# nkkrnkl/category-agnostic-pose-estimation

Hardware: AMD Instinct MI355X
Metric: episodes/sec (1-shot, 256x256, 17kpt) training step (higher is better)
Workload: dtype f32 storage/accumulate, GEMMs as bf16x3 split (3 bf16 MFMAs per product); 1 GPU; configs[1]: 1-shot training step (fwd+loss+bwd+clip+AdamW at learning rate 0, dropout on), 256x256, 17 kpt, ResNet-50 + deformable transformer, 16 episodes x 2 queries per GPU; episodes_per_gpu=16, queries_per_episode=2, image_size=256, global_batch_episodes=16, parallelism=dp1, weights=random init (no checkpoint offline)

## Files before the change

category-agnostic-pose-estimation_amd/hip/functional.py:

```python
import contextlib
import ctypes
import os

import torch

from . import lib, ops


class Runtime:
    rng = None
    direct_grad = False
    use_side_stream = os.environ.get("CAPE_SIDE_STREAM", "1") == "1"
    side = None
    on_param_grad = []
    capture_keep = None

    pending = []
    side_dirty = False

    defer_wgrad = os.environ.get("CAPE_DEFER_WGRAD", "1") == "1"
    wgrad_group = int(os.environ.get("CAPE_WGRAD_GROUP", "12"))
    wq = {}
    wq_total = 0
    wq_notify = []
# ... 1059 lines not shown
        ref = _c(ref)
        ctx.save_for_backward(ref)
        return ops.query_sine_fwd(ref).view(*ref.shape[:-1], 256)

    @staticmethod
    def backward(ctx, d_out):
        (ref,) = ctx.saved_tensors
        return ops.query_sine_bwd(_c(d_out).view(-1, 256), ref).view_as(ref)


def query_sine(ref):
    return QuerySineFn.apply(ref)


class RefineFn(torch.autograd.Function):
    @staticmethod
    def forward(ctx, delta, ref):
        delta, ref = _c(delta), _c(ref)
        out = ops.refine_fwd(delta, ref)
        ctx.save_for_backward(out, ref)
        return out

    @staticmethod
    def backward(ctx, d_new):
        out, ref = ctx.saved_tensors
        d_delta, d_ref = ops.refine_bwd(_c(d_new), out, ref)
        return d_delta, d_ref


def refine(delta, ref):
    return RefineFn.apply(delta, ref)


class SigmoidFn(torch.autograd.Function):
    @staticmethod
    def forward(ctx, x):
        y = ops.sigmoid_fwd(_c(x))
        ctx.save_for_backward(y)
        return y

    @staticmethod
    def backward(ctx, dy):
        (y,) = ctx.saved_tensors
        return ops.sigmoid_bwd(_c(dy), y)


def sigmoid(x):
    return SigmoidFn.apply(x)


class RefScaleFn(torch.autograd.Function):

    @staticmethod
    def forward(ctx, ref, valid_ratios):
        ref, vr = _c(ref), _c(valid_ratios)
        N, Lq, _ = ref.shape
        L = vr.shape[1]
        ctx.save_for_backward(vr)
        ctx.meta = (N, Lq, L)
        return ops.ref_scale_fwd(ref, vr, Lq, L).view(N, Lq, L, 2)

    @staticmethod
    def backward(ctx, d):
        (vr,) = ctx.saved_tensors
        N, Lq, L = ctx.meta
        return ops.ref_scale_bwd(_c(d), vr, Lq, L).view(N, Lq, 2), None
# ... 193 lines not shown
```

category-agnostic-pose-estimation_amd/hip/lib.py:

```python
import ctypes
import os

import torch

from ctypes import POINTER, c_char_p, c_float, c_int, c_int32, c_int64, c_longlong, c_size_t, c_uint32, c_uint64, c_uint8, c_void_p

_HERE = os.path.dirname(os.path.abspath(__file__))
LIB_PATH = os.environ.get("CAPE_HIP_LIB", os.path.join(_HERE, "..", "csrc", "libcape_hip.so"))
LIB_PATH = os.path.abspath(LIB_PATH)

if not os.path.exists(LIB_PATH):
    raise ImportError(
        f"libcape_hip.so not found at {LIB_PATH}; build it with `python -c 'import __graft_entry__ as g; g.build()'` "
        "(or `make -C category-agnostic-pose-estimation_amd/csrc`).  There is no CPU fallback.")
try:
    _lib = ctypes.CDLL(LIB_PATH)
except OSError as e:
    raise ImportError(f"cannot load {LIB_PATH}: {e}") from e

_lib.cape_last_error.restype = c_char_p
_lib.cape_abi_version.restype = c_int


class GemmDesc(ctypes.Structure):
# ... 100 lines not shown
    "cape_msda_bwd": [P, P, P, P, P, P, P, P, P, I, I, I, I, I, P],
    "cape_msda_bwd_ex": [P, P, P, P, P, P, P, P, P, I, I, I, I, I, I, P],
    "cape_msda_bwd_atomic": [P, P, P, P, P, P, P, P, P, I, I, I, I, I, P],
    "cape_attn_fwd": [P, P, P, P, P, LL, LL, LL, LL, LL, LL, LL, LL, I, I, I, I, F, I, I, P, F, P, U32, P],
    "cape_attn_bwd": [P, P, P, P, P, P, P, P, P, LL, LL, LL, LL, LL, LL, LL, LL, I, I, I, I, F, I, I, P, F, P, U32, P],
    "cape_flash_attn_fwd": [P, P, P, P, P, LL, LL, LL, LL, LL, LL, LL, LL, I, I, I, I, F, I, I, P, F, P, U32, P],
    "cape_flash_attn_bwd": [P, P, P, P, P, P, P, P, P, P, LL, LL, LL, LL, LL, LL, LL, LL, I, I, I, I, F, I, I, P, F, P, U32, P],
    "cape_attn_softmax_fwd": [P, P, P, I, I, I, I, F, I, I, P, F, P, U32, P],
    "cape_attn_softmax_bwd": [P, P, I, I, I, I, F, F, P, U32, P],
    "cape_add_f32": [P, P, P, LL, P],
    "cape_level_embed_add": [P, P, P, P, I, I, I, I, P],
    "cape_add_n_f32": [POINTER(c_void_p), I, P, LL, P],
    "cape_add_n_rows_f32": [POINTER(c_void_p), POINTER(c_longlong), I, P, LL, LL, I, P],
    "cape_augment_batch": [P, I, I, I, P, P, P],
    "cape_gelu_f32": [P, P, LL, P],
    "cape_support_masks": [P, P, P, I, I, I, P],
    "cape_interleave2x2_f32": [POINTER(c_void_p), P, P, I, I, I, I, P],
    "cape_gelu_bwd_f32": [P, P, P, LL, P],
    "cape_scale_residual_bwd_f32": [P, P, P, P, P, LL, I, P],
    "cape_scale_residual_f32": [P, P, P, P, LL, I, P],
    "cape_nchw_to_nhwc": [P, P, I, I, I, I, I, P],
    "cape_bn_fold": [P, P, P, P, F, P, P, I, P],
    "cape_maxpool3x3s2_nhwc": [P, P, I, I, I, I, P],
    "cape_bn_relu_bwd": [P, P, P, P, P, LL, I, I, P],
    "cape_affine_act_f32": [P, P, P, P, LL, I, I, P],
    "cape_relu_drop_bwd": [P, P, P, LL, F, P],
    "cape_pos_sine_level": [P, P, P, P, LL, I, I, I, I, P],
    "cape_token_embed_fwd": [P, P, P, P, P, P, P, P, P, P, LL, I, I, P],
    "cape_token_embed_bwd": [P, P, P, P, P, P, P, P, P, P, LL, I, I, I, P],
    "cape_query_sine_fwd": [P, P, P, LL, P],
    "cape_query_sine_bwd": [P, P, P, P, I, LL, P],
    "cape_refine_fwd": [P, P, P, LL, P],
    "cape_refine_bwd": [P, P, P, P, P, I, LL, P],
    "cape_sigmoid_fwd": [P, P, LL, P],
    "cape_sigmoid_bwd": [P, P, P, I, LL, P],
    "cape_ref_scale_fwd": [P, P, P, LL, I, I, P],
    "cape_ref_scale_bwd": [P, P, P, I, LL, I, I, P],
    "cape_support_embed_fwd": [P, P, P, P, P, P, P, I, I, I, P],
    "cape_support_embed_bwd": [P, P, P, P, P, I, I, I, P],
    "cape_adjacency": [P, P, P, P, I, I, P],
    "cape_gcn_aggregate_fwd": [P, P, P, I, I, I, P],
    "cape_gcn_aggregate_bwd": [P, P, P, P, I, I, I, P],
    "cape_zero_rows": [P, P, LL, I, P],
    "cape_legacy_coord_embed_fwd": [P, P, P, P, I, I, P],
    "cape_legacy_coord_embed_bwd": [P, P, P, P, P, P, P, I, I, P],
    "cape_support_edge_info_fwd": [P, P, P, P, LL, P, P, P, I, I, I, P],
    "cape_support_edge_info_bwd": [P, LL, P, P, P, I, I, P],
    "cape_pe_dropout_fwd": [P, P, P, I, I, I, F, P, U32, P],
    "cape_pe_dropout_bwd": [P, P, LL, F, P, U32, P],
    "cape_loss_fwd_bwd": [P, P, P, P, P, P, F, F, F, P, P, P, P, I, LL, P],
    "cape_sumsq": [P, LL, P, P],
    "cape_adamw_step": [P, P, P, P, LL, F, F, F, F, F, F, P, I, P, P, P],
    "cape_step_increment": [P, P],
    "cape_step_guard": [P, P, I, P, I, F, P, P, P, P, P, I, I, P],
    "cape_adamw_step_guarded": [P, P, P, P, LL, F, F, F, F, F, F, P, I, P, P, P, P],
    "cape_decode_next_tokens": [P, P, P, P, P, P, I, I, I, I, I, I, P],
    "cape_decode_advance": [P, LL, P, LL, P, P, P, I, I, I, I, I, I, I, P, I, I, P, P, P],
    "cape_decode_linear": [POINTER(DecodeLinearDesc), P],
    "cape_decode_tail": [POINTER(DecodeTailDesc), P],
    "cape_decode_step": [POINTER(DecodeStepDesc), P],
}
EXPORTS = ["cape_last_error", "cape_abi_version", "cape_groupnorm_workspace_bytes", "cape_packed_weight_bytes"] + list(_SIGS)
_lib.cape_packed_weight_bytes.argtypes = [I, I]
_lib.cape_packed_weight_bytes.restype = c_size_t
_lib.cape_groupnorm_workspace_bytes.argtypes = [I, I, I]
_lib.cape_groupnorm_workspace_bytes.restype = c_size_t
# ... 24 lines not shown
```

category-agnostic-pose-estimation_amd/hip/ops.py:

```python
import ctypes
import math
import os
import weakref

import torch

from . import lib

_F32 = torch.float32


_raw_stream = getattr(torch._C, "_cuda_getCurrentRawStream", None)
_raw_device = getattr(torch._C, "_cuda_getDevice", None)


_side = [None]


def raw_current_stream():
    if _raw_stream is not None and _raw_device is not None:
        return _raw_stream(_raw_device())
    return torch.cuda.current_stream().cuda_stream


# ... 552 lines not shown
         batch=(N * H, H, Q.stride(0), 32, K.stride(0), 32, H * Lq * Lk, Lq * Lk))
    P = torch.empty_like(S)
    Pd = torch.empty_like(S) if dropout_p > 0 else None
    lib.call("cape_attn_softmax_fwd", _p(S), _p(P), _p(Pd), N, H, Lq, Lk, float(scale), mask_mode, causal_offset, _p(kpm),
             float(dropout_p), _rng_ptr(rng, dropout_p), rng_stream, _stream())
    Pu = Pd if Pd is not None else P
    O = torch.empty(N, Lq, H * 32, dtype=_F32, device=dev)
    gemm(Pu, V, O, Lq, 32, Lk, a_mode=0, b_mode=1, lda=Lk, ldb=_ld(V), ldc=H * 32,
         batch=(N * H, H, H * Lq * Lk, Lq * Lk, V.stride(0), 32, Lq * H * 32, 32))
    return O, P, Pu


def attn_mm_bwd(dO, Q, K, V, P, Pu, dQ, dK, dV, N, H, Lq, Lk, scale, dropout_p=0.0, rng=None, rng_stream=0):
    blk, img = Lq * Lk, H * Lq * Lk
    gemm(Pu, dO, dV, Lk, 32, Lq, a_mode=1, b_mode=1, lda=Lk, ldb=H * 32, ldc=_ld(dV),
         batch=(N * H, H, img, blk, Lq * H * 32, 32, dV.stride(0), 32))
    dS = torch.empty(N, H, Lq, Lk, dtype=_F32, device=dO.device)
    gemm(dO, V, dS, Lq, Lk, 32, lda=H * 32, ldb=_ld(V), ldc=Lk,
         batch=(N * H, H, Lq * H * 32, 32, V.stride(0), 32, img, blk))
    lib.call("cape_attn_softmax_bwd", _p(P), _p(dS), N, H, Lq, Lk, float(scale), float(dropout_p),
             _rng_ptr(rng, dropout_p), rng_stream, _stream())
    gemm(dS, K, dQ, Lq, 32, Lk, a_mode=0, b_mode=1, lda=Lk, ldb=_ld(K), ldc=_ld(dQ),
         batch=(N * H, H, img, blk, K.stride(0), 32, dQ.stride(0), 32))
    gemm(dS, Q, dK, Lk, 32, Lq, a_mode=1, b_mode=1, lda=Lk, ldb=_ld(Q), ldc=_ld(dK),
         batch=(N * H, H, img, blk, Q.stride(0), 32, dK.stride(0), 32))


def attn_route(N, H, Lq, Lk, flash=False):
    if flash and flash_attn_ok(N, H, Lq, Lk):
        return "flash"
    return "mm" if attn_mm_ok(N, H, Lq, Lk) else "scalar"


_ATTN_LAUNCHERS = {"scalar": (attn_fwd, attn_bwd), "flash": (flash_attn_fwd, flash_attn_bwd)}


def attn_core_fwd(route, Q, K, V, N, H, Lq, Lk, scale, mask_mode=0, causal_offset=0, kpm=None, dropout_p=0.0, rng=None, rng_stream=0):
    if route == "mm":
        O, P, Pu = attn_mm_fwd(Q, K, V, N, H, Lq, Lk, scale, mask_mode, causal_offset, kpm, dropout_p, rng, rng_stream)
        return O, (P, Pu)
    O, lse = _ATTN_LAUNCHERS[route][0](Q, K, V, N, H, Lq, Lk, scale, mask_mode, causal_offset, kpm, dropout_p, rng, rng_stream)
    return O, (lse,)


def attn_core_bwd(route, saved, dO, Q, K, V, O, dQ, dK, dV, N, H, Lq, Lk, scale, mask_mode=0, causal_offset=0, kpm=None, dropout_p=0.0,
                  rng=None, rng_stream=0):
    if route == "mm":
        attn_mm_bwd(dO, Q, K, V, *saved, dQ, dK, dV, N, H, Lq, Lk, scale, dropout_p, rng, rng_stream)
    else:
        _ATTN_LAUNCHERS[route][1](dO, Q, K, V, O, *saved, dQ, dK, dV, N, H, Lq, Lk, scale, mask_mode, causal_offset, kpm, dropout_p,
                                  rng, rng_stream)


def add(a, b):
    _chk(a, "add.a"); _chk(b, "add.b")
    assert a.shape == b.shape
    out = torch.empty_like(a)
    lib.call("cape_add_f32", _p(a), _p(b), _p(out), a.numel(), _stream())
    return out


def add_n(tensors):
    k = len(tensors)
    assert 1 <= k <= 8
    for t in tensors:
        _chk(t, "add_n.src")
# ... 206 lines not shown
    R = seqs[0].numel()
    lib.call("cape_token_embed_bwd", _p(d_out), *[_p(s) for s in seqs], *[_p(d) for d in deltas], _p(d_table), R, C, V,
             int(pad_idx), _stream())


def query_sine_fwd(ref):
    _chk(ref, "qsine.ref")
    R = ref.numel() // 2
    out = torch.empty(R, 256, dtype=_F32, device=ref.device)
    lib.call("cape_query_sine_fwd", _p(ref), _p(dim_t(ref.device)), _p(out), R, _stream())
    return out


def query_sine_bwd(d_out, ref):
    _chk(d_out, "qsine_bwd.d_out")
    d_ref = torch.empty_like(ref)
    lib.call("cape_query_sine_bwd", _p(d_out), _p(ref), _p(dim_t(ref.device)), _p(d_ref), 0, ref.numel() // 2, _stream())
    return d_ref


def refine_fwd(delta, ref):
    _chk(delta, "refine.delta"); _chk(ref, "refine.ref")
    assert delta.shape == ref.shape
    out = torch.empty_like(ref)
    lib.call("cape_refine_fwd", _p(delta), _p(ref), _p(out), ref.numel(), _stream())
    return out


def refine_bwd(d_new, new_ref, ref):
    _chk(d_new, "refine_bwd.d_new")
    d_delta, d_ref = torch.empty_like(ref), torch.empty_like(ref)
    lib.call("cape_refine_bwd", _p(d_new), _p(new_ref), _p(ref), _p(d_delta), _p(d_ref), 0, ref.numel(), _stream())
    return d_delta, d_ref


def sigmoid_fwd(x):
    _chk(x, "sigmoid.x")
    y = torch.empty_like(x)
    lib.call("cape_sigmoid_fwd", _p(x), _p(y), x.numel(), _stream())
    return y


def sigmoid_bwd(dy, y):
    _chk(dy, "sigmoid_bwd.dy")
    dx = torch.empty_like(y)
    lib.call("cape_sigmoid_bwd", _p(dy), _p(y), _p(dx), 0, y.numel(), _stream())
    return dx


def ref_scale_fwd(ref, valid_ratios, rows_per_image, L):
    _chk(ref, "ref_scale.ref"); _chk(valid_ratios, "ref_scale.vr")
    R = ref.numel() // 2
    out = torch.empty(R, L, 2, dtype=_F32, device=ref.device)
    lib.call("cape_ref_scale_fwd", _p(ref), _p(valid_ratios), _p(out), R, rows_per_image, L, _stream())
    return out


def ref_scale_bwd(d_in, valid_ratios, rows_per_image, L):
    _chk(d_in, "ref_scale_bwd.d_in")
    R = d_in.numel() // (2 * L)
    d_ref = torch.empty(R, 2, dtype=_F32, device=d_in.device)
    lib.call("cape_ref_scale_bwd", _p(d_in), _p(valid_ratios), _p(d_ref), 0, R, rows_per_image, L, _stream())
    return d_ref


def support_embed_fwd(coords, W0, b0, pe1d, N, P, C=256):
# ... 368 lines not shown
```

category-agnostic-pose-estimation_amd/models/deformable_transformer_v2.py:

```python
import copy
import math
import os

import numpy as np
import torch
from torch import nn
from torch.nn.init import normal_

from ..hip import functional as HF
from ..hip import ops
from .deformable_transformer import (DeformableTransformerEncoder, DeformableTransformerEncoderLayer, MSDeformAttn)
from ..util.misc import cached_zero_mask
from .kv_cache import KVCache, VCache

_ONES_VR = {}
_FUSED_SELF_ATTN = os.environ.get("CAPE_DEC_SELF_ATTN_NODE", "1") == "1"


def Embedding(num_embeddings, embedding_dim, padding_idx=None, zero_init=False):
    m = nn.Embedding(num_embeddings, embedding_dim, padding_idx=padding_idx)
    nn.init.normal_(m.weight, mean=0, std=embedding_dim ** -0.5)
    if padding_idx is not None:
        nn.init.constant_(m.weight[padding_idx], 0)
    if zero_init:
# ... 149 lines not shown
        return HF.token_embed(self.token_embed.weight, self.pad_idx, seq11, seq21, seq12, seq22,
                              delta_x1, delta_x2, delta_y1, delta_y2)

    def _query_pos(self, reference_points):
        qs = HF.query_sine(reference_points)
        qp = HF.linear(qs, self.pos_trans.weight, self.pos_trans.bias)
        return HF.add_layernorm(qp, None, self.pos_trans_norm.weight, self.pos_trans_norm.bias)

    def _mlp(self, mlp, x):
        n = len(mlp.layers)
        for i, layer in enumerate(mlp.layers):
            x = HF.linear(x, layer.weight, layer.bias, relu=(i < n - 1))
        return x

    def forward(self, reference_points, src, geo, src_valid_ratios, padding_rows_u8=None, seq_kwargs=None,
                support_features=None, support_mask=None):
        if support_features is None:
            support_features = getattr(self, "support_features", None)
        if support_mask is None:
            support_mask = getattr(self, "support_mask", None)
        kpm = ops.as_u8(support_mask) if (support_features is not None and support_mask is not None) else None
        output = self._seq_embed(seq11=seq_kwargs["seq11"], seq12=seq_kwargs["seq12"], seq21=seq_kwargs["seq21"],
                                 seq22=seq_kwargs["seq22"], delta_x1=seq_kwargs["delta_x1"], delta_x2=seq_kwargs["delta_x2"],
                                 delta_y1=seq_kwargs["delta_y1"], delta_y2=seq_kwargs["delta_y2"])
        hs, refs, clss = [], [], []
        nl = len(self.layers)
        mems = HF.fanout(src, nl)
        sups = HF.fanout(support_features, nl) if support_features is not None else (None,) * nl
        for lid, layer in enumerate(self.layers):
            r_scale, r_sine, r_ref = HF.fanout(reference_points, 3)
            ref_in = HF.ref_scale(r_scale, src_valid_ratios)
            query_pos = self._query_pos(r_sine)
            output = layer(output, query_pos, ref_in, mems[lid], geo, padding_rows_u8, sups[lid], kpm)
            o_mlp, o_cls, o_hs, output = HF.fanout(output, 4)
            delta = self._mlp(self.coords_embed[lid], o_mlp)
            reference_points, r_keep = HF.fanout(HF.refine(delta, r_ref), 2)
            cls = HF.linear(o_cls, self.class_embed[lid].weight, self.class_embed[lid].bias)
            hs.append(o_hs); refs.append(r_keep); clss.append(cls)
        return hs, torch.stack(refs), torch.stack(clss)

    @torch.no_grad()
    def decode_step(self, tok, delta, ref_step, geo, valid_ratios, step, caches):
        N = tok.shape[1]
        output = ops.token_embed_fwd(self.token_embed.weight, [tok[0], tok[2], tok[1], tok[3]],
                                     [delta[0], delta[1], delta[2], delta[3]]).view(N, 1, -1)
        ref = ref_step
        for lid, layer in enumerate(self.layers):
            ref_in = ops.ref_scale_fwd(ref, valid_ratios, 1, geo.L).view(N, 1, geo.L, 2)
            qs = ops.query_sine_fwd(ref)
            qp = torch.empty(N, 256, dtype=torch.float32, device=ref.device)
            ops.gemm(qs, self.pos_trans.weight, qp, N, 256, 256, bias=self.pos_trans.bias)
            qp, _, _, _ = ops.add_layernorm_fwd(qp, None, self.pos_trans_norm.weight, self.pos_trans_norm.bias)
            output = layer.decode_step(output, qp.view(N, 1, 256), ref_in, geo, step, caches[lid])
            x = output.view(N, 256)
            mlp = self.coords_embed[lid].layers
            for i, l in enumerate(mlp):
                y = torch.empty(N, l.weight.shape[0], dtype=torch.float32, device=x.device)
                ops.gemm(x, l.weight, y, N, l.weight.shape[0], l.weight.shape[1], bias=l.bias, relu=(i < len(mlp) - 1))
                x = y
            ref = ops.refine_fwd(x.view(N, 1, 2), ref)
        ce = self.class_embed[-1]
        cls = torch.empty(N, ce.weight.shape[0], dtype=torch.float32, device=ref.device)
        ops.gemm(output.view(N, 256), ce.weight, cls, N, ce.weight.shape[0], 256, bias=ce.bias)
        return output, ref, cls


class DeformableTransformer(nn.Module):
    def __init__(self, d_model=256, nhead=8, num_encoder_layers=6, num_decoder_layers=6, dim_feedforward=1024, dropout=0.1,
                 activation="relu", poly_refine=True, return_intermediate_dec=False, aux_loss=False, num_feature_levels=4,
                 dec_n_points=4, enc_n_points=4, query_pos_type="none", vocab_size=None, seq_len=1024,
# ... 87 lines not shown
```

include/cape_hip.h:

```cpp
#ifndef CAPE_HIP_H
#define CAPE_HIP_H

#include <stddef.h>
#include <stdint.h>

#ifdef __cplusplus
extern "C" {
#endif

typedef void* cape_stream_t;

const char* cape_last_error(void);
int cape_abi_version(void);

int cape_rng_advance(uint64_t* rng_state, cape_stream_t stream);

int cape_stream_fork(cape_stream_t main_stream, cape_stream_t side_stream);
int cape_stream_join(cape_stream_t main_stream, cape_stream_t side_stream);

typedef struct {
  int M, N, K;
  int a_mode, b_mode;
  const float* A; long long lda;
  const float* B; long long ldb;
// ... 166 lines not shown
int cape_scale_residual_f32(const float* x, const float* y, const float* gamma, float* out, long long rows, int C,
                            cape_stream_t stream);
int cape_gelu_bwd_f32(const float* x, const float* g, float* dx, long long n, cape_stream_t stream);
int cape_scale_residual_bwd_f32(const float* g, const float* y, const float* gamma, float* dy, float* dgamma, long long rows, int C,
                                cape_stream_t stream);
int cape_nchw_to_nhwc(const float* x, float* out, int N, int C, int H, int W, int Cp, cape_stream_t stream);
int cape_bn_fold(const float* w, const float* b, const float* rm, const float* rv, float eps,
                 float* scale, float* shift, int C, cape_stream_t stream);
int cape_maxpool3x3s2_nhwc(const float* x, float* out, int N, int H, int W, int C, cape_stream_t stream);
int cape_bn_relu_bwd(const float* dy, const float* y, const float* scale, float* d_pre, float* d_res,
                     long long rows, int C, int relu, cape_stream_t stream);
int cape_affine_act_f32(float* x, const float* scale, const float* bias, const float* residual, long long rows, int C, int relu,
                        cape_stream_t stream);
int cape_relu_drop_bwd(const float* dh, const float* h, float* d_pre, long long n, float inv_keep,
                       cape_stream_t stream);
int cape_pos_sine_level(const uint8_t* mask, const float* level_embed_l, const float* dim_t, float* out,
                        long long out_image_stride, int N, int h, int w, int C, cape_stream_t stream);

int cape_token_embed_fwd(const float* table, const int64_t* s11, const int64_t* s21, const int64_t* s12,
                         const int64_t* s22, const float* dx1, const float* dx2, const float* dy1,
                         const float* dy2, float* out, long long R, int C, int vocab, cape_stream_t stream);
int cape_token_embed_bwd(const float* d_out, const int64_t* s11, const int64_t* s21, const int64_t* s12,
                         const int64_t* s22, const float* dx1, const float* dx2, const float* dy1,
                         const float* dy2, float* d_table, long long R, int C, int vocab, int pad_idx,
                         cape_stream_t stream);

int cape_query_sine_fwd(const float* ref, const float* dim_t, float* out, long long R, cape_stream_t stream);
int cape_query_sine_bwd(const float* d_out, const float* ref, const float* dim_t, float* d_ref, int accumulate, long long R,
                        cape_stream_t stream);

int cape_refine_fwd(const float* delta, const float* ref, float* new_ref, long long n, cape_stream_t stream);
int cape_refine_bwd(const float* d_new, const float* new_ref, const float* ref, float* d_delta,
                    float* d_ref, int accumulate_ref, long long n, cape_stream_t stream);
int cape_sigmoid_fwd(const float* x, float* y, long long n, cape_stream_t stream);
int cape_sigmoid_bwd(const float* dy, const float* y, float* dx, int accumulate, long long n,
                     cape_stream_t stream);
int cape_ref_scale_fwd(const float* ref, const float* valid_ratios, float* ref_in, long long R,
                       int rows_per_image, int L, cape_stream_t stream);
int cape_ref_scale_bwd(const float* d_ref_in, const float* valid_ratios, float* d_ref, int accumulate,
                       long long R, int rows_per_image, int L, cape_stream_t stream);

int cape_support_embed_fwd(const float* coords, const float* W0, const float* b0, const float* pe1d,
                           const float* dim_t, float* h, float* pe, int N, int P, int C, cape_stream_t stream);
int cape_support_embed_bwd(const float* d_h, const float* h, const float* coords, float* dW0, float* db0,
                           int N, int P, int C, cape_stream_t stream);
int cape_adjacency(const int* edges, const int* edge_start, const uint8_t* mask, float* adj, int N, int P,
                   cape_stream_t stream);
int cape_support_masks(const uint8_t* mask, uint8_t* kpm, uint8_t* zero, int N, int P, int pad_rows, cape_stream_t stream);
int cape_gcn_aggregate_fwd(const float* y, const float* adj, float* out, int N, int P, int C,
                           cape_stream_t stream);
int cape_gcn_aggregate_bwd(const float* d_out, const float* out, const float* adj, float* d_y, int N,
                           int P, int C, cape_stream_t stream);
int cape_zero_rows(float* x, const uint8_t* rowmask, long long rows, int C, cape_stream_t stream);

int cape_legacy_coord_embed_fwd(const float* coords, const float* W0, const float* b0, float* h, int R, int C, cape_stream_t stream);
int cape_legacy_coord_embed_bwd(const float* d_h, const float* h, const float* coords, const float* W0, float* dW0, float* db0,
                                float* d_coords, int R, int C, cape_stream_t stream);
int cape_support_edge_info_fwd(const int* edges, const int* edge_start, const float* E, float* out, long long ldo, float* scale,
                               uint8_t* has, float* deg, int N, int P, int C, cape_stream_t stream);
int cape_support_edge_info_bwd(const float* g, long long ldg, const float* scale, const uint8_t* has, float* dE, int R, int C,
                               cape_stream_t stream);
int cape_pe_dropout_fwd(const float* x, const float* pe, float* out, int R, int P, int C, float dropout_p, const uint64_t* rng_state,
                        uint32_t rng_stream, cape_stream_t stream);
int cape_pe_dropout_bwd(const float* g, float* dx, long long total, float dropout_p, const uint64_t* rng_state, uint32_t rng_stream,
                        cape_stream_t stream);

// ... 54 lines not shown
```

Measured before the change: 648.3 episodes/s.

## Fuse decoder coord MLP, refine and class heads into single kernels

Adds fused HIP forward and backward kernels that run the decoder's per-layer 3-layer coordinate MLP, the inverse-sigmoid refine, and the class linear head in one launch each. Activations stay in LDS as bf16 hi/lo planes between the MFMA stages instead of going through separate GEMM and elementwise launches. The goal is to cut per-layer launch count and intermediate global memory traffic. It adds routing logic and packed-weight lookup, and small-weight gradients are summed with atomics.

```diff
diff --git a/category-agnostic-pose-estimation_amd/csrc/dec_chain.hip b/category-agnostic-pose-estimation_amd/csrc/dec_chain.hip
--- /dev/null
+++ b/category-agnostic-pose-estimation_amd/csrc/dec_chain.hip
@@ -0,0 +1,407 @@
+#include "gemm_common.h"
+
+namespace {
+
+constexpr int DC_UNIT = 64;
+constexpr int DC_C = 256;
+constexpr int DC_KS = DC_C / 16;
+constexpr int DC_LD = DC_C + 8;
+constexpr int DC_PLANE = DC_UNIT * DC_LD;
+constexpr int DC_IMG = 2 * DC_PLANE;
+constexpr int DC_FLD = DC_C + 4;
+constexpr int DC_SMALL = DC_UNIT * 8 + 5 * DC_C;
+constexpr size_t DC_LDS_BYTES = (size_t)2 * DC_IMG * 2 + (size_t)DC_SMALL * 4;
+static_assert((size_t)DC_UNIT * DC_FLD * 4 <= (size_t)DC_IMG * 2, "an fp32 unit fits in one image");
+static_assert(DC_LDS_BYTES <= 160 * 1024, "LDS of one CU");
+
+#define DC_PIN() asm volatile("" ::: "memory")
+__device__ __forceinline__ unsigned dc_opaque_zero() {
+  unsigned z = 0;
+  asm volatile("" : "+s"(z));
+  return z;
+}
+
+__device__ __forceinline__ int roff16(int i) { return (i & 3) + 8 * (i >> 2); }
+
+__device__ __forceinline__ void load_frags(bf16x8 (&bhi)[DC_KS], bf16x8 (&blo)[DC_KS], const unsigned short* pack, int grp, int lane) {
+  const char* bp = reinterpret_cast<const char*>(pack) + ((size_t)grp * (DC_KS * 2 * 1024) + dc_opaque_zero());
+  const unsigned lo = 16u * (unsigned)lane;
+#pragma unroll
+  for (int s = 0; s < DC_KS; ++s) {
+    bhi[s] = __builtin_bit_cast(bf16x8, *reinterpret_cast<const uint4*>(bp + (2 * s + 0) * 1024 + lo));
+    blo[s] = __builtin_bit_cast(bf16x8, *reinterpret_cast<const uint4*>(bp + (2 * s + 1) * 1024 + lo));
+  }
+}
+
+__device__ __forceinline__ f32x16 stage_mma(const unsigned short* img, int half, int r, int h, const bf16x8 (&bhi)[DC_KS],
+                                            const bf16x8 (&blo)[DC_KS], int single) {
+  f32x16 acc;
+#pragma unroll
+  for (int i = 0; i < 16; ++i) acc[i] = 0.f;
+  const unsigned short* Ah = img + (32 * half + r) * DC_LD + 8 * h;
+  const unsigned short* Al = Ah + DC_PLANE;
+#pragma unroll
+  for (int s = 0; s < DC_KS; ++s) {
+    const bf16x8 ahi = *reinterpret_cast<const bf16x8*>(Ah + 16 * s);
+    const bf16x8 alo = *reinterpret_cast<const bf16x8*>(Al + 16 * s);
+    if (!single) {
+      acc = __builtin_amdgcn_mfma_f32_32x32x16_bf16(alo, bhi[s], acc, 0, 0, 0);
+      acc = __builtin_amdgcn_mfma_f32_32x32x16_bf16(ahi, blo[s], acc, 0, 0, 0);
+    }
+    acc = __builtin_amdgcn_mfma_f32_32x32x16_bf16(ahi, bhi[s], acc, 0, 0, 0);
+  }
+  return acc;
+}
+
+__device__ __forceinline__ void put_piece(unsigned short* img, int row, int kc, float4 v) {
+  unsigned short* Ph = img + row * DC_LD + 4 * kc;
+  unsigned h0, l0, h1, l1;
+  split2(v.x, v.y, h0, l0);
+  split2(v.z, v.w, h1, l1);
+  *reinterpret_cast<uint2*>(Ph) = make_uint2(h0, h1);
+  *reinterpret_cast<uint2*>(Ph + DC_PLANE) = make_uint2(l0, l1);
+}
+
+__device__ __forceinline__ void put_pair(unsigned short* img, int row, int col, float v0, float v1) {
+  unsigned hi, lo;
+  split2(v0, v1, hi, lo);
+  unsigned short* Ph = img + row * DC_LD + col;
+  Ph[0] = (unsigned short)(hi & 0xffffu);
+  Ph[DC_LD] = (unsigned short)(hi >> 16);
+  Ph[DC_PLANE] = (unsigned short)(lo & 0xffffu);
+  Ph[DC_PLANE + DC_LD] = (unsigned short)(lo >> 16);
+}
+
+__device__ __forceinline__ float dc_inv_sigmoid(float x) {
+  x = fminf(fmaxf(x, 0.f), 1.f);
+  const float x1 = fmaxf(x, 1e-5f), x2 = fmaxf(1.f - x, 1e-5f);
+  return logf(x1 / x2);
+}
+
+__device__ __forceinline__ float dot4(const float4& a, const float4& b) {
+  return fmaf(a.w, b.w, fmaf(a.z, b.z, fmaf(a.y, b.y, a.x * b.x)));
+}
+
+struct HeadsFwdP {
+  int M, single;
+  const float* x; const float* ref;
+  const unsigned short* w1p; const float* b1;
+  const unsigned short* w2p; const float* b2;
+  const float* w3; const float* b3;
+  const float* wc; const float* bc;
+  float* h1; float* h2; float* new_ref; float* cls;
+};
+
+__global__ void __launch_bounds__(512) dec_heads_fwd_kernel(const HeadsFwdP p) {
+  extern __shared__ __attribute__((aligned(16))) unsigned short lds[];
+  unsigned short* img0 = lds;
+  unsigned short* img1 = lds + DC_IMG;
+  const int t = threadIdx.x, lane = t & 63, wave = __builtin_amdgcn_readfirstlane(t >> 6);
+  const int r = lane & 31, h = lane >> 5;
+  const int col = 32 * wave + r;
+  const unsigned lo_c = (unsigned)(4 * h * DC_C + col);
+  const int nunits = (p.M + DC_UNIT - 1) / DC_UNIT;
+
+  const float b1 = p.b1[col], b2 = p.b2[col];
+  float4 wc[3];
+#pragma unroll
+  for (int c = 0; c < 3; ++c) wc[c] = *reinterpret_cast<const float4*>(p.wc + c * DC_C + 4 * lane);
+  const float bcv = lane < 3 ? p.bc[lane] : 0.f;
+
+  for (int u = blockIdx.x; u < nunits; u += gridDim.x) {
+    const int row0 = u * DC_UNIT;
+    bf16x8 bhi[DC_KS], blo[DC_KS];
+    float4 ra[8];
+#pragma unroll
+    for (int i = 0; i < 8; ++i) {
+      const int row = min(row0 + wave + 8 * i, p.M - 1);
+      ra[i] = *reinterpret_cast<const float4*>(p.x + (long long)row * DC_C + 4 * lane);
+    }
+    load_frags(bhi, blo, p.w1p, wave, lane);
+#pragma unroll
+    for (int i = 0; i < 8; ++i) {
+      const int row = row0 + wave + 8 * i;
+      const float s0 = wave_sum(dot4(ra[i], wc[0]));
+      const float s1 = wave_sum(dot4(ra[i], wc[1]));
+      const float s2 = wave_sum(dot4(ra[i], wc[2]));
+      const float s = lane == 0 ? s0 : lane == 1 ? s1 : s2;
+      if (lane < 3 && row < p.M) p.cls[(long long)row * 3 + lane] = s + bcv;
+    }
+#pragma unroll
+    for (int i = 0; i < 8; ++i) put_piece(img0, wave + 8 * i, lane, ra[i]);
+    __syncthreads();
+
+#pragma unroll 1
+    for (int half = 0; half < 2; ++half) {
+      const f32x16 acc = stage_mma(img0, half, r, h, bhi, blo, p.single);
+      const int lrow = 32 * half + 4 * h;
+      float* c0 = p.h1 + (long long)(row0 + 32 * half) * DC_C;
+      const int rlim = p.M - row0 - lrow;
+#pragma unroll
+      for (int i = 0; i < 16; i += 2) {
+        const int ro = roff16(i);
+        float v0 = fmaxf(fmaf(acc[i], 1.f, b1), 0.f), v1 = fmaxf(fmaf(acc[i + 1], 1.f, b1), 0.f);
+        if (ro < rlim) c0[lo_c + (unsigned)(ro * DC_C)] = v0;
+        if (ro + 1 < rlim) c0[lo_c + (unsigned)((ro + 1) * DC_C)] = v1;
+        put_pair(img1, lrow + ro, col, v0, v1);
+      }
+    }
+    DC_PIN();
+    load_frags(bhi, blo, p.w2p, wave, lane);
+    __syncthreads();
+
+    float* F = reinterpret_cast<float*>(img0);
+#pragma unroll 1
+    for (int half = 0; half < 2; ++half) {
+      const f32x16 acc = stage_mma(img1, half, r, h, bhi, blo, p.single);
+      const int lrow = 32 * half + 4 * h;
+      float* c0 = p.h2 + (long long)(row0 + 32 * half) * DC_C;
+      const int rlim = p.M - row0 - lrow;
+#pragma unroll
+      for (int i = 0; i < 16; ++i) {
+        const int ro = roff16(i);
+        const float v = fmaxf(fmaf(acc[i], 1.f, b2), 0.f);
+        if (ro < rlim) c0[lo_c + (unsigned)(ro * DC_C)] = v;
+        F[(lrow + ro) * DC_FLD + col] = v;
+      }
+    }
+    __syncthreads();
+
+    {
+      const int lrow = t >> 3, part = t & 7;
+      float s0 = 0.f, s1 = 0.f;
+      const float* w3 = p.w3 + dc_opaque_zero();
+#pragma unroll
+      for (int j = 0; j < 8; ++j) {
+        const int k = 4 * part + 32 * j;
+        const float4 hv = *reinterpret_cast<const float4*>(F + lrow * DC_FLD + k);
+        const float4 w0 = *reinterpret_cast<const float4*>(w3 + k);
+        const float4 w1 = *reinterpret_cast<const float4*>(w3 + DC_C + k);
+        s0 += dot4(hv, w0);
+        s1 += dot4(hv, w1);
+      }
+      s0 += cape_dpp<0xB1>(s0); s0 += cape_dpp<0x4E>(s0); s0 += cape_dpp<0x141>(s0);
+      s1 += cape_dpp<0xB1>(s1); s1 += cape_dpp<0x4E>(s1); s1 += cape_dpp<0x141>(s1);
+      const int row = row0 + lrow;
+      if (part < 2 && row < p.M) {
+        const long long o = (long long)row * 2 + part;
+        const float z = (part == 0 ? s0 : s1) + p.b3[part] + dc_inv_sigmoid(p.ref[o]);
+        p.new_ref[o] = 1.f / (1.f + expf(-z));
+      }
+    }
+    __syncthreads();
+  }
+}
+
+struct HeadsBwdP {
+  int M, single, acc_dx;
+  const float* d_new; const float* d_cls; const float* new_ref; const float* ref;
+  const float* x; const float* h1; const float* h2;
+  const unsigned short* w2tp; const unsigned short* w1tp;
+  const float* w3; const float* wc;
+  float* dpre2; float* dpre1; float* d_x; float* d_ref;
+  float* dw3; float* db3; float* dwc; float* dbc;
+};
+
+__global__ void __launch_bounds__(512) dec_heads_bwd_kernel(const HeadsBwdP p) {
+  extern __shared__ __attribute__((aligned(16))) unsigned short lds[];
+  unsigned short* img0 = lds;
+  unsigned short* img1 = lds + DC_IMG;
+  float* sdz = reinterpret_cast<float*>(lds + 2 * DC_IMG);
+  float* sdc = sdz + 2 * DC_UNIT;
+  const int t = threadIdx.x, lane = t & 63, wave = __builtin_amdgcn_readfirstlane(t >> 6);
+  const int r = lane & 31, h = lane >> 5;
+  const int col = 32 * wave + r;
+  const unsigned lo_c = (unsigned)(4 * h * DC_C + col);
+  const int nunits = (p.M + DC_UNIT - 1) / DC_UNIT;
+
+  const float wc0 = p.wc[col], wc1 = p.wc[DC_C + col], wc2 = p.wc[2 * DC_C + col];
+  float* wsum = sdz + DC_UNIT * 8;
+  for (int e = t; e < 5 * DC_C; e += 512) wsum[e] = 0.f;
+  float pb = 0.f;
+
+  for (int u = blockIdx.x; u < nunits; u += gridDim.x) {
+    const int row0 = u * DC_UNIT;
+    bf16x8 bhi[DC_KS], blo[DC_KS];
+    if (t < 2 * DC_UNIT) {
+      const int row = row0 + (t >> 1);
+      float dz = 0.f;
+      if (row < p.M) {
+        const long long o = (long long)row * 2 + (t & 1);
+        const float s = p.new_ref[o];
+        dz = p.d_new[o] * s * (1.f - s);
+        const float x = p.ref[o];
+        float dx = 0.f;
+        if (x >= 0.f && x <= 1.f) {
+          if (x >= 1e-5f) dx += 1.f / x;
+          if (1.f - x >= 1e-5f) dx += 1.f / (1.f - x);
+        }
+        p.d_ref[o] = dz * dx;
+      }
+      sdz[t] = dz;
+      pb += dz;
+    } else if (t < 2 * DC_UNIT + 4 * DC_UNIT) {
+      const int q = t - 2 * DC_UNIT, lrow = q >> 2, c = q & 3;
+      const int row = row0 + lrow;
+      const float v = (c < 3 && row < p.M) ? p.d_cls[(long long)row * 3 + c] : 0.f;
+      sdc[q] = v;
+      pb += v;
+    }
+    __syncthreads();
+
+    const float* w3 = p.w3 + dc_opaque_zero();
+    const float4 w30 = *reinterpret_cast<const float4*>(w3 + 4 * lane);
+    const float4 w31 = *reinterpret_cast<const float4*>(w3 + DC_C + 4 * lane);
+    float4 pw[5];
+#pragma unroll
+    for (int q = 0; q < 5; ++q) pw[q] = zero4();
+#pragma unroll
+    for (int i = 0; i < 8; ++i) {
+      const int lrow = wave + 8 * i;
+      const int row = row0 + lrow, crow = min(row, p.M - 1);
+      const float4 hv = *reinterpret_cast<const float4*>(p.h2 + (long long)crow * DC_C + 4 * lane);
+      const float4 xv = *reinterpret_cast<const float4*>(p.x + (long long)crow * DC_C + 4 * lane);
+      const float dz0 = sdz[2 * lrow], dz1 = sdz[2 * lrow + 1];
+      const float dc0 = sdc[4 * lrow], dc1 = sdc[4 * lrow + 1], dc2 = sdc[4 * lrow + 2];
+      float4 g;
+      g.x = hv.x > 0.f ? fmaf(dz1, w31.x, dz0 * w30.x) : 0.f;
+      g.y = hv.y > 0.f ? fmaf(dz1, w31.y, dz0 * w30.y) : 0.f;
+      g.z = hv.z > 0.f ? fmaf(dz1, w31.z, dz0 * w30.z) : 0.f;
+      g.w = hv.w > 0.f ? fmaf(dz1, w31.w, dz0 * w30.w) : 0.f;
+      pw[0].x = fmaf(dz0, hv.x, pw[0].x); pw[0].y = fmaf(dz0, hv.y, pw[0].y); pw[0].z = fmaf(dz0, hv.z, pw[0].z); pw[0].w = fmaf(dz0, hv.w, pw[0].w);
+      pw[1].x = fmaf(dz1, hv.x, pw[1].x); pw[1].y = fmaf(dz1, hv.y, pw[1].y); pw[1].z = fmaf(dz1, hv.z, pw[1].z); pw[1].w = fmaf(dz1, hv.w, pw[1].w);
+      pw[2].x = fmaf(dc0, xv.x, pw[2].x); pw[2].y = fmaf(dc0, xv.y, pw[2].y); pw[2].z = fmaf(dc0, xv.z, pw[2].z); pw[2].w = fmaf(dc0, xv.w, pw[2].w);
+      pw[3].x = fmaf(dc1, xv.x, pw[3].x); pw[3].y = fmaf(dc1, xv.y, pw[3].y); pw[3].z = fmaf(dc1, xv.z, pw[3].z); pw[3].w = fmaf(dc1, xv.w, pw[3].w);
+      pw[4].x = fmaf(dc2, xv.x, pw[4].x); pw[4].y = fmaf(dc2, xv.y, pw[4].y); pw[4].z = fmaf(dc2, xv.z, pw[4].z); pw[4].w = fmaf(dc2, xv.w, pw[4].w);
+      if (row < p.M) *reinterpret_cast<float4*>(p.dpre2 + (long long)row * DC_C + 4 * lane) = g;
+      put_piece(img0, lrow, lane, g);
+    }
+#pragma unroll
+    for (int q = 0; q < 5; ++q) {
+      float* w = wsum + q * DC_C + 4 * lane;
+      atomicAdd(w, pw[q].x); atomicAdd(w + 1, pw[q].y); atomicAdd(w + 2, pw[q].z); atomicAdd(w + 3, pw[q].w);
+    }
+    DC_PIN();
+    load_frags(bhi, blo, p.w2tp, wave, lane);
+    __syncthreads();
+
+#pragma unroll 1
+    for (int half = 0; half < 2; ++half) {
+      const int lrow = 32 * half + 4 * h;
+      const int rlim = p.M - row0 - lrow;
+      float gate[16];
+#pragma unroll
+      for (int i = 0; i < 16; ++i) {
+        const int row = min(row0 + lrow + roff16(i), p.M - 1);
+        gate[i] = p.h1[(unsigned)(row * DC_C + col)];
+      }
+      const f32x16 acc = stage_mma(img0, half, r, h, bhi, blo, p.single);
+      float* c0 = p.dpre1 + (long long)(row0 + 32 * half) * DC_C;
+#pragma unroll
+      for (int i = 0; i < 16; i += 2) {
+        const int ro = roff16(i);
+        float v0 = gate[i] != 0.f ? acc[i] : 0.f, v1 = gate[i + 1] != 0.f ? acc[i + 1] : 0.f;
+        if (ro < rlim) c0[lo_c + (unsigned)(ro * DC_C)] = v0;
+        if (ro + 1 < rlim) c0[lo_c + (unsigned)((ro + 1) * DC_C)] = v1;
+        put_pair(img1, lrow + ro, col, v0, v1);
+      }
+    }
+    DC_PIN();
+    load_frags(bhi, blo, p.w1tp, wave, lane);
+    __syncthreads();
+
+#pragma unroll 1
+    for (int half = 0; half < 2; ++half) {
+      const int lrow = 32 * half + 4 * h;
+      const int rlim = p.M - row0 - lrow;
+      float* c0 = p.d_x + (long long)(row0 + 32 * half) * DC_C;
+      const f32x16 acc = stage_mma(img1, half, r, h, bhi, blo, p.single);
+      DC_PIN();
+      float old[16];
+#pragma unroll
+      for (int i = 0; i < 16; ++i) {
+        const int ro = roff16(i);
+        old[i] = (p.acc_dx && ro < rlim) ? c0[lo_c + (unsigned)(ro * DC_C)] : 0.f;
+      }
+#pragma unroll
+      for (int i = 0; i < 16; ++i) {
+        const int ro = roff16(i);
+        const float* dc = sdc + 4 * (lrow + ro);
+        const float v = acc[i] + fmaf(dc[2], wc2, fmaf(dc[1], wc1, dc[0] * wc0)) + old[i];
+        if (ro < rlim) c0[lo_c + (unsigned)(ro * DC_C)] = v;
+      }
+    }
+    __syncthreads();
+  }
+
+  if (t < 6 * DC_UNIT) sdz[t] = pb;
+  __syncthreads();
+  if (wave < 5) {
+    const float s = wave_sum(wave < 2 ? sdz[2 * lane + wave] : sdc[4 * lane + (wave - 2)]);
+    if (lane == 0) atomicAdd(wave < 2 ? p.db3 + wave : p.dbc + (wave - 2), s);
+  }
+  for (int e = t; e < 5 * DC_C; e += 512) atomicAdd(e < 2 * DC_C ? p.dw3 + e : p.dwc + (e - 2 * DC_C), wsum[e]);
+}
+
+int set_lds_attr(const void* kfn, bool& done, const char* name) {
+  if (done) return 0;
+  hipError_t e = hipFuncSetAttribute(kfn, hipFuncAttributeMaxDynamicSharedMemorySize, (int)DC_LDS_BYTES);
+  if (e != hipSuccess) return cape_set_error("%s: hipFuncSetAttribute: %s", name, hipGetErrorString(e));
+  done = true;
+  return 0;
+}
+
+bool al16(const void* q) { return (reinterpret_cast<uintptr_t>(q) & 15) == 0; }
+
+}
+
+extern "C" int cape_dec_heads_fwd(const float* x, const float* ref, const void* w1_packed, const float* b1, const void* w2_packed,
+                                  const float* b2, const float* w3, const float* b3, const float* wc, const float* bc, float* h1,
+                                  float* h2, float* new_ref, float* cls, int rows, int single, cape_stream_t stream) {
+  CAPE_REQUIRE(x && ref && w1_packed && b1 && w2_packed && b2 && w3 && b3 && wc && bc && h1 && h2 && new_ref && cls,
+               "cape_dec_heads_fwd: null pointer");
+  CAPE_REQUIRE(rows >= 0 && rows < (1 << 22), "cape_dec_heads_fwd: rows=%d out of range", rows);
+  CAPE_REQUIRE(al16(x) && al16(w1_packed) && al16(w2_packed) && al16(w3) && al16(wc),
+               "cape_dec_heads_fwd: x, the packed weights, w3 and wc must be 16-byte aligned");
+  if (rows == 0) return 0;
+  static bool attr = false;
+  if (int rc = set_lds_attr(reinterpret_cast<const void*>(dec_heads_fwd_kernel), attr, "cape_dec_heads_fwd")) return rc;
+  HeadsFwdP p;
+  p.M = rows; p.single = single != 0;
+  p.x = x; p.ref = ref;
+  p.w1p = static_cast<const unsigned short*>(w1_packed); p.b1 = b1;
+  p.w2p = static_cast<const unsigned short*>(w2_packed); p.b2 = b2;
+  p.w3 = w3; p.b3 = b3; p.wc = wc; p.bc = bc;
+  p.h1 = h1; p.h2 = h2; p.new_ref = new_ref; p.cls = cls;
+  const int nunits = (rows + DC_UNIT - 1) / DC_UNIT;
+  hipLaunchKernelGGL(dec_heads_fwd_kernel, dim3((unsigned)(nunits < 256 ? nunits : 256)), dim3(512), DC_LDS_BYTES, as_stream(stream), p);
+  CAPE_LAUNCH_CHECK("cape_dec_heads_fwd");
+  return 0;
+}
+
+extern "C" int cape_dec_heads_bwd(const float* d_new_ref, const float* d_cls, const float* new_ref, const float* ref, const float* x,
+                                  const float* h1, const float* h2, const void* w2t_packed, const void* w1t_packed, const float* w3,
+                                  const float* wc, float* dpre2, float* dpre1, float* d_x, int accumulate_dx, float* d_ref, float* dw3,
+                                  float* db3, float* dwc, float* dbc, int rows, int single, cape_stream_t stream) {
+  CAPE_REQUIRE(d_new_ref && d_cls && new_ref && ref && x && h1 && h2 && w2t_packed && w1t_packed && w3 && wc && dpre2 && dpre1 && d_x &&
+                   d_ref && dw3 && db3 && dwc && dbc,
+               "cape_dec_heads_bwd: null pointer");
+  CAPE_REQUIRE(rows >= 0 && rows < (1 << 22), "cape_dec_heads_bwd: rows=%d out of range", rows);
+  CAPE_REQUIRE(al16(x) && al16(h2) && al16(dpre2) && al16(w2t_packed) && al16(w1t_packed) && al16(w3),
+               "cape_dec_heads_bwd: x, h2, dpre2, the packed weights and w3 must be 16-byte aligned");
+  if (rows == 0) return 0;
+  static bool attr = false;
+  if (int rc = set_lds_attr(reinterpret_cast<const void*>(dec_heads_bwd_kernel), attr, "cape_dec_heads_bwd")) return rc;
+  HeadsBwdP p;
+  p.M = rows; p.single = single != 0; p.acc_dx = accumulate_dx != 0;
+  p.d_new = d_new_ref; p.d_cls = d_cls; p.new_ref = new_ref; p.ref = ref;
+  p.x = x; p.h1 = h1; p.h2 = h2;
+  p.w2tp = static_cast<const unsigned short*>(w2t_packed); p.w1tp = static_cast<const unsigned short*>(w1t_packed);
+  p.w3 = w3; p.wc = wc;
+  p.dpre2 = dpre2; p.dpre1 = dpre1; p.d_x = d_x; p.d_ref = d_ref;
+  p.dw3 = dw3; p.db3 = db3; p.dwc = dwc; p.dbc = dbc;
+  const int nunits = (rows + DC_UNIT - 1) / DC_UNIT;
+  hipLaunchKernelGGL(dec_heads_bwd_kernel, dim3((unsigned)(nunits < 256 ? nunits : 256)), dim3(512), DC_LDS_BYTES, as_stream(stream), p);
+  CAPE_LAUNCH_CHECK("cape_dec_heads_bwd");
+  return 0;
+}
diff --git a/category-agnostic-pose-estimation_amd/hip/functional.py b/category-agnostic-pose-estimation_amd/hip/functional.py
--- a/category-agnostic-pose-estimation_amd/hip/functional.py
+++ b/category-agnostic-pose-estimation_amd/hip/functional.py
@@ -1115,6 +1115,60 @@
     return RefineFn.apply(delta, ref)
 
 
+class DecHeadsFn(torch.autograd.Function):
+
+    @staticmethod
+    def forward(ctx, x, ref, w1, b1, w2, b2, w3, b3, wc, bc):
+        x2, ref2 = _c(x).view(-1, 256), _c(ref).view(-1, 2)
+        packs = ops.dec_heads_packs(w1, w2, 0)
+        if packs is None:
+            raise RuntimeError("DecHeadsFn: packed weight planes are missing (ask dec_heads_route before building the node)")
+        h1, h2, new_ref, cls = ops.dec_heads_fwd(x2, ref2, packs, b1, b2, _c(w3), b3, _c(wc), bc)
+        ctx.save_for_backward(x2, ref2, h1, h2, new_ref, w1, w2, w3, wc)
+        ctx.refs = (w1, b1, w2, b2, w3, b3, wc, bc)
+        ctx.slot = _slot_of(x)
+        ctx.xshape, ctx.rshape = x.shape, ref.shape
+        return new_ref.view(ref.shape), cls.view(*x.shape[:-1], 3)
+
+    @staticmethod
+    def backward(ctx, d_new_ref, d_cls):
+        x2, ref2, h1, h2, new_ref, w1, w2, w3, wc = ctx.saved_tensors
+        R, dev = x2.shape[0], x2.device
+        packs_t = ops.dec_heads_packs(w1, w2, 1)
+        if packs_t is None:
+            raise RuntimeError("DecHeadsFn: packed dgrad weight planes are missing")
+        pg = _ParamGrads(ctx.refs, ctx.needs_input_grad[2:10])
+        dw1, db1, dw2, db2 = pg.bufs[:4]
+        dw3, db3, dwc, dbc = (b if b is not None else torch.zeros_like(r) for b, r in zip(pg.bufs[4:], ctx.refs[4:]))
+        dx, acc = _grad_target(ctx.slot, (R, 256), dev)
+        d_ref, dpre1, dpre2 = ops.dec_heads_bwd(_c(d_new_ref), _c(d_cls), new_ref, ref2, x2, h1, h2, packs_t, _c(w3), _c(wc),
+                                                dx, acc, dw3, db3, dwc, dbc)
+        with pg.side(dpre1, dpre2, x2, h1):
+            for dpre, a, dw, db in ((dpre1, x2, dw1, db1), (dpre2, h1, dw2, db2)):
+                if dw is not None:
+                    pg.gemm(dpre, a, dw, 256, 256, R, a_mode=1, b_mode=1, lda=256, ldb=256, ldc=dw.stride(0), accumulate=True,
+                            split_k=ops.pick_split_k(256, 256, R), colsum_out=db)
+                elif db is not None:
+                    ops.colsum(dpre, R, 256, db)
+        return (dx.view(ctx.xshape), d_ref.view(ctx.rshape)) + pg.result()
+
+
+def dec_heads_route(coords_mlp, class_linear, rows):
+    ls = list(coords_mlp.layers)
+    shapes = [tuple(l.weight.shape) for l in ls] + [tuple(class_linear.weight.shape)]
+    if shapes != [(256, 256), (256, 256), (2, 256), (3, 256)] or any(l.bias is None for l in ls + [class_linear]):
+        return "nodes"
+    if ops.dec_chain_route(256, True, rows) != "chain" or not ls[0].weight.is_cuda:
+        return "nodes"
+    w1, w2 = ls[0].weight, ls[1].weight
+    return ops.dec_chain_route(256, ops.dec_heads_packs(w1, w2, 0) is not None and ops.dec_heads_packs(w1, w2, 1) is not None, rows)
+
+
+def dec_heads(x, ref, coords_mlp, class_linear):
+    l1, l2, l3 = coords_mlp.layers
+    return DecHeadsFn.apply(x, ref, l1.weight, l1.bias, l2.weight, l2.bias, l3.weight, l3.bias, class_linear.weight, class_linear.bias)
+
+
 class SigmoidFn(torch.autograd.Function):
     @staticmethod
     def forward(ctx, x):
diff --git a/category-agnostic-pose-estimation_amd/hip/lib.py b/category-agnostic-pose-estimation_amd/hip/lib.py
--- a/category-agnostic-pose-estimation_amd/hip/lib.py
+++ b/category-agnostic-pose-estimation_amd/hip/lib.py
@@ -156,6 +156,8 @@
     "cape_query_sine_bwd": [P, P, P, P, I, LL, P],
     "cape_refine_fwd": [P, P, P, LL, P],
     "cape_refine_bwd": [P, P, P, P, P, I, LL, P],
+    "cape_dec_heads_fwd": [P] * 14 + [I, I, P],
+    "cape_dec_heads_bwd": [P] * 14 + [I] + [P] * 5 + [I, I, P],
     "cape_sigmoid_fwd": [P, P, LL, P],
     "cape_sigmoid_bwd": [P, P, P, I, LL, P],
     "cape_ref_scale_fwd": [P, P, P, LL, I, I, P],
diff --git a/category-agnostic-pose-estimation_amd/hip/ops.py b/category-agnostic-pose-estimation_amd/hip/ops.py
--- a/category-agnostic-pose-estimation_amd/hip/ops.py
+++ b/category-agnostic-pose-estimation_amd/hip/ops.py
@@ -608,6 +608,15 @@
     return "mm" if attn_mm_ok(N, H, Lq, Lk) else "scalar"
 
 
+_DEC_CHAIN = os.environ.get("CAPE_DEC_CHAIN", "1") != "0"
+
+
+def dec_chain_route(hidden, packed_ok, rows, precision=None, enabled=None):
+    precision = GEMM_PRECISION if precision is None else _PRECISIONS[precision]
+    enabled = _DEC_CHAIN if enabled is None else enabled
+    return "chain" if (enabled and precision >= 1 and hidden == 256 and packed_ok and rows > 64) else "nodes"
+
+
 _ATTN_LAUNCHERS = {"scalar": (attn_fwd, attn_bwd), "flash": (flash_attn_fwd, flash_attn_bwd)}
 
 
@@ -880,6 +889,52 @@
     d_delta, d_ref = torch.empty_like(ref), torch.empty_like(ref)
     lib.call("cape_refine_bwd", _p(d_new), _p(new_ref), _p(ref), _p(d_delta), _p(d_ref), 0, ref.numel(), _stream())
     return d_delta, d_ref
+
+
+def dec_heads_packs(w1, w2, b_mode):
+    if not PackedWeights.enabled or tuple(w1.shape) != (256, 256) or tuple(w2.shape) != (256, 256):
+        return None
+    packs = tuple(PackedWeights.lookup(w, 256, 256, w.stride(0), b_mode) if w.stride(1) == 1 else None for w in (w1, w2))
+    return None if any(q is None for q in packs) else packs
+
+
+def _chk_packed(q, name):
+    assert q.dtype == torch.int16 and q.is_cuda and q.numel() * 2 >= lib.raw().cape_packed_weight_bytes(256, 256), name
+
+
+def dec_heads_fwd(x, ref, packs, b1, b2, w3, b3, wc, bc):
+    for t, n in ((x, "x"), (ref, "ref"), (b1, "b1"), (b2, "b2"), (w3, "w3"), (b3, "b3"), (wc, "wc"), (bc, "bc")):
+        _chk(t, "dec_heads." + n)
+    R = x.shape[0]
+    assert x.shape == (R, 256) and ref.numel() == 2 * R and R < (1 << 22)
+    assert b1.numel() == 256 and b2.numel() == 256 and w3.shape == (2, 256) and b3.numel() == 2 and wc.shape == (3, 256) and bc.numel() == 3
+    _chk_packed(packs[0], "dec_heads.w1_packed"); _chk_packed(packs[1], "dec_heads.w2_packed")
+    h1 = torch.empty(R, 256, dtype=_F32, device=x.device)
+    h2 = torch.empty(R, 256, dtype=_F32, device=x.device)
+    new_ref = torch.empty(R, 2, dtype=_F32, device=x.device)
+    cls = torch.empty(R, 3, dtype=_F32, device=x.device)
+    lib.call("cape_dec_heads_fwd", _p(x), _p(ref), _p(packs[0]), _p(b1), _p(packs[1]), _p(b2), _p(w3), _p(b3), _p(wc), _p(bc),
+             _p(h1), _p(h2), _p(new_ref), _p(cls), R, int(GEMM_PRECISION == 2), _stream())
+    return h1, h2, new_ref, cls
+
+
+def dec_heads_bwd(d_new_ref, d_cls, new_ref, ref, x, h1, h2, packs_t, w3, wc, d_x, acc_dx, dw3, db3, dwc, dbc):
+    for t, n in ((d_new_ref, "d_new_ref"), (d_cls, "d_cls"), (new_ref, "new_ref"), (ref, "ref"), (x, "x"), (h1, "h1"), (h2, "h2"),
+                 (w3, "w3"), (wc, "wc"), (d_x, "d_x"), (dw3, "dw3"), (db3, "db3"), (dwc, "dwc"), (dbc, "dbc")):
+        _chk(t, "dec_heads_bwd." + n)
+    R = x.shape[0]
+    assert x.shape == (R, 256) and h1.shape == (R, 256) and h2.shape == (R, 256) and d_x.numel() == R * 256 and R < (1 << 22)
+    assert d_new_ref.numel() == 2 * R and new_ref.numel() == 2 * R and ref.numel() == 2 * R and d_cls.numel() == 3 * R
+    assert w3.shape == (2, 256) and wc.shape == (3, 256) and dw3.shape == (2, 256) and dwc.shape == (3, 256)
+    assert db3.numel() == 2 and dbc.numel() == 3
+    _chk_packed(packs_t[0], "dec_heads_bwd.w1t_packed"); _chk_packed(packs_t[1], "dec_heads_bwd.w2t_packed")
+    dpre1 = torch.empty(R, 256, dtype=_F32, device=x.device)
+    dpre2 = torch.empty(R, 256, dtype=_F32, device=x.device)
+    d_ref = torch.empty(R, 2, dtype=_F32, device=x.device)
+    lib.call("cape_dec_heads_bwd", _p(d_new_ref), _p(d_cls), _p(new_ref), _p(ref), _p(x), _p(h1), _p(h2), _p(packs_t[1]), _p(packs_t[0]),
+             _p(w3), _p(wc), _p(dpre2), _p(dpre1), _p(d_x), int(bool(acc_dx)), _p(d_ref), _p(dw3), _p(db3), _p(dwc), _p(dbc),
+             R, int(GEMM_PRECISION == 2), _stream())
+    return d_ref, dpre1, dpre2
 
 
 def sigmoid_fwd(x):
diff --git a/category-agnostic-pose-estimation_amd/models/deformable_transformer_v2.py b/category-agnostic-pose-estimation_amd/models/deformable_transformer_v2.py
--- a/category-agnostic-pose-estimation_amd/models/deformable_transformer_v2.py
+++ b/category-agnostic-pose-estimation_amd/models/deformable_transformer_v2.py
@@ -205,10 +205,14 @@
             ref_in = HF.ref_scale(r_scale, src_valid_ratios)
             query_pos = self._query_pos(r_sine)
             output = layer(output, query_pos, ref_in, mems[lid], geo, padding_rows_u8, sups[lid], kpm)
-            o_mlp, o_cls, o_hs, output = HF.fanout(output, 4)
-            delta = self._mlp(self.coords_embed[lid], o_mlp)
-            reference_points, r_keep = HF.fanout(HF.refine(delta, r_ref), 2)
-            cls = HF.linear(o_cls, self.class_embed[lid].weight, self.class_embed[lid].bias)
+            if HF.dec_heads_route(self.coords_embed[lid], self.class_embed[lid], output.numel() // output.shape[-1]) == "chain":
+                o_heads, o_hs, output = HF.fanout(output, 3)
+                new_ref, cls = HF.dec_heads(o_heads, r_ref, self.coords_embed[lid], self.class_embed[lid])
+            else:
+                o_mlp, o_cls, o_hs, output = HF.fanout(output, 4)
+                new_ref = HF.refine(self._mlp(self.coords_embed[lid], o_mlp), r_ref)
+                cls = HF.linear(o_cls, self.class_embed[lid].weight, self.class_embed[lid].bias)
+            reference_points, r_keep = HF.fanout(new_ref, 2)
             hs.append(o_hs); refs.append(r_keep); clss.append(cls)
         return hs, torch.stack(refs), torch.stack(clss)
 
diff --git a/include/cape_hip.h b/include/cape_hip.h
--- a/include/cape_hip.h
+++ b/include/cape_hip.h
@@ -222,6 +222,14 @@
 int cape_refine_fwd(const float* delta, const float* ref, float* new_ref, long long n, cape_stream_t stream);
 int cape_refine_bwd(const float* d_new, const float* new_ref, const float* ref, float* d_delta,
                     float* d_ref, int accumulate_ref, long long n, cape_stream_t stream);
+
+int cape_dec_heads_fwd(const float* x, const float* ref, const void* w1_packed, const float* b1, const void* w2_packed,
+                       const float* b2, const float* w3, const float* b3, const float* wc, const float* bc, float* h1,
+                       float* h2, float* new_ref, float* cls, int rows, int single, cape_stream_t stream);
+int cape_dec_heads_bwd(const float* d_new_ref, const float* d_cls, const float* new_ref, const float* ref, const float* x,
+                       const float* h1, const float* h2, const void* w2t_packed, const void* w1t_packed, const float* w3,
+                       const float* wc, float* dpre2, float* dpre1, float* d_x, int accumulate_dx, float* d_ref, float* dw3,
+                       float* db3, float* dwc, float* dbc, int rows, int single, cape_stream_t stream);
 int cape_sigmoid_fwd(const float* x, float* y, long long n, cape_stream_t stream);
 int cape_sigmoid_bwd(const float* dy, const float* y, float* dx, int accumulate, long long n,
                      cape_stream_t stream);
```

Measured after the change: 666.6 episodes/s, median of 4. 2.8% higher.
